# robotseu/ORB_Line_SLAM

Hardware: AMD Instinct MI355X
Metric: stereo frames/s extract+match (ORB+LBD), KITTI 1242x375 (higher is better)
Workload: dtype u8; 1 GPU; C3: 1242x375 stereo, 2000 ORB + 500 LBD per image, extract + stereo point/line match + f2f LBD match + SearchByBoW vs the previous frame (synthetic k=10 L=6 vocabulary, ComputeBoW included); parallelism=frame-sharded x1, distinct_pairs=512, order=shuffled, scene=default

## Files before the change

### orb_line_slam_amd/csrc/api.cpp

```cpp
#include "ctx.hpp"
#include "staging.hpp"
#include <map>
#include <mutex>

namespace olf {
static thread_local std::string g_err;
void set_error(const std::string& s) { g_err = s; }

int check_device(const olf_ctx* c, const char* who)
{
    int d = -1;
    if (hipGetDevice(&d) != hipSuccess || d != c->device) { set_error(std::string(who) + ": the context belongs to another device than the current one"); return OLF_ERR_INVALID; }
    return OLF_OK;
}

int scratch_get(olf_ctx* c, ScratchSlot slot, size_t bytes, void** out)
{
    if (c->scratch_bytes[slot] < bytes) {
        if (c->scratch[slot]) { OLF_HIP_CHECK(hipDeviceSynchronize()); (void)hipFree(c->scratch[slot]); c->scratch[slot] = nullptr; c->scratch_bytes[slot] = 0; }
        size_t want = std::max<size_t>(bytes * 3 / 2, 4096);
        OLF_HIP_CHECK(hipMalloc(&c->scratch[slot], want));
        c->scratch_bytes[slot] = want;
    }
    *out = c->scratch[slot];
// ... 171 lines not shown
    if (c->ev_join) (void)hipEventDestroy(c->ev_join);
    if (c->stream2) (void)hipStreamDestroy(c->stream2);
    if (c->stream) (void)hipStreamDestroy(c->stream);
    delete c;
}

int olf_ctx_create(const olf_params* p, int width, int height, int max_images, olf_ctx** out)
{
    if (!p || !out || width < 64 || height < 64 || max_images < 1) { set_error("olf_ctx_create: bad argument"); return OLF_ERR_INVALID; }
    *out = nullptr;
    if (p->abi_version != OLF_ABI_VERSION || p->struct_size != (uint32_t)sizeof(olf_params)) {
        set_error("olf_ctx_create: the parameter block was not initialised by this library's olf_default_params() (abi_version / struct_size differ: "
                  "caller built against another include/orbline_types.h)");
        return OLF_ERR_INVALID;
    }
    int ndev = 0;
    if (hipGetDeviceCount(&ndev) != hipSuccess || ndev < 1) {
        set_error("olf_ctx_create: no HIP device visible (this library has no CPU path)");
        return OLF_ERR_NODEVICE;
    }
    olf_ctx* c = new olf_ctx();
    c->params = *p; c->W = width; c->H = height; c->max_images = max_images;
    int rc = c->orb.build(p->orb, width, height);
    if (rc != OLF_OK) {
        set_error(rc == OLF_ERR_CAPACITY ? "olf_ctx_create: more than 32760 key points on one pyramid level (nfeatures too large for this scale factor / level count)"
                  : (width > kMaxOrbSide || height > kMaxOrbSide) ? "olf_ctx_create: image wider or higher than 4131 pixels (FAST candidates are packed with 12 bits per coordinate)"
                                         : "olf_ctx_create: image size / ORB parameters not supported (every pyramid level needs at least 62 x 62 pixels and a landscape cell grid)");
        delete c; return rc;
    }
    auto fail = [&](int code) { olf_ctx_destroy(c); return code; };
    if (hipGetDevice(&c->device) != hipSuccess) return fail(OLF_ERR_HIP);
    if (hipDeviceGetAttribute(&c->limits.nCU, hipDeviceAttributeMultiprocessorCount, c->device) != hipSuccess || c->limits.nCU <= 0) c->limits.nCU = 64;
    if (hipDeviceGetAttribute(&c->limits.maxLds, hipDeviceAttributeMaxSharedMemoryPerBlock, c->device) != hipSuccess) c->limits.maxLds = 64 * 1024;
    if (hipStreamCreateWithFlags(&c->stream, hipStreamNonBlocking) != hipSuccess) { set_error("hipStreamCreate failed"); return fail(OLF_ERR_HIP); }
    const OrbGeom& g = c->orb.geom;
    const size_t n = (size_t)max_images;
    OrbDeviceBufs& b = c->ob;
    const bool allocTrace = getenv("OLF_ALLOC_TRACE") != nullptr;
#define A(ptr, count) do { if ((rc = dev_alloc(c, &(ptr), (count))) != OLF_OK) return fail(rc); \
                           if (allocTrace) fprintf(stderr, "alloc %-18s %8.3f MB per image\n", #ptr, (double)(count) * sizeof(*(ptr)) / 1e6 / (double)n); } while (0)
    A(b.pyr, n * g.pyrBytes); A(b.blur, n * g.pyrBytes);
    A(b.cells, n * g.totalCells * g.cellCap); A(b.cellCount, n * g.totalCells);
    A(b.cand, n * g.candTotal); A(b.candNode, n * g.candTotal); A(b.candCount, n * g.nlevels);
    if (g.maxNodes > 2048) A(b.octSpill, n * g.nlevels * octree_lds_bytes(g.maxNodes));
    A(b.lvlKp, n * g.kpTotal); A(b.lvlCount, n * g.nlevels); A(b.lvlAngle, n * g.kpTotal);
    A(b.rx, c->orb.rx.size() + 1); A(b.ry, c->orb.ry.size() + 1); A(b.geom, 1); A(b.status, 256);
    A(c->d_sad, ((n + 1) / 2) * g.outCap); A(c->d_bestkey, ((n + 1) / 2) * g.outCap); A(c->d_rowperm, n * g.outCap);
    A(c->d_images, n * width * height);
#undef A
    if (hipMemcpy(b.rx, c->orb.rx.data(), c->orb.rx.size() * sizeof(ResizeCoef), hipMemcpyHostToDevice) != hipSuccess ||
        hipMemcpy(b.ry, c->orb.ry.data(), c->orb.ry.size() * sizeof(ResizeCoef), hipMemcpyHostToDevice) != hipSuccess ||
        hipMemcpy(b.geom, &g, sizeof(OrbGeom), hipMemcpyHostToDevice) != hipSuccess ||
        hipMemset(b.status, 0, 1024) != hipSuccess) {
        set_error("olf_ctx_create: table upload failed");
        return fail(OLF_ERR_HIP);
    }
    rc = c->line.build(p->line, width, height, max_images);
    if (rc != OLF_OK) { set_error("olf_ctx_create: LSD parameters not supported"); return fail(rc); }
    LineGeom& lg = c->line.geom;
    int prLeast = 0, prGreatest = 0;
    (void)hipDeviceGetStreamPriorityRange(&prLeast, &prGreatest);
    if (hipStreamCreateWithPriority(&c->stream2, hipStreamNonBlocking, prLeast) != hipSuccess ||
        hipEventCreateWithFlags(&c->ev_fork, hipEventDisableTiming) != hipSuccess || hipEventCreateWithFlags(&c->ev_front, hipEventDisableTiming) != hipSuccess || hipEventCreateWithFlags(&c->ev_sort, hipEventDisableTiming) != hipSuccess ||
        hipEventCreateWithFlags(&c->ev_lbd, hipEventDisableTiming) != hipSuccess ||
        hipEventCreateWithFlags(&c->ev_join, hipEventDisableTiming) != hipSuccess) { set_error("stream/event creation failed"); return fail(OLF_ERR_HIP); }
    LineDeviceBufs& l = c->lb;
#define A(ptr, count) do { if ((rc = dev_alloc(c, &(ptr), (count))) != OLF_OK) return fail(rc); \
                           if (allocTrace) fprintf(stderr, "alloc %-18s %8.3f MB per image\n", #ptr, (double)(count) * sizeof(*(ptr)) / 1e6 / (double)n); } while (0)
    const bool batchCtx = n > (size_t)kBatchCtxImages;
    const size_t keyWords = lg.wide ? 2 : 1;
    A(l.grad, n * lg.Ps); A(l.keysA, n * lg.Ps * keyWords); A(l.keysB, n * lg.Ps * keyWords);
    if (batchCtx && lg.Ps * 4 >= lg.pitchW * lg.H && lg.Ps * 4 >= lg.pitchS * lg.Hs) { l.lsdBlur = reinterpret_cast<uint8_t*>(l.keysA); l.scaled = reinterpret_cast<uint8_t*>(l.keysB); c->scaled_aliased = true; }
    else { A(l.lsdBlur, n * lg.pitchW * lg.H); A(l.scaled, n * lg.pitchS * lg.Hs); }
    A(l.topBuf, n * (size_t)lsd_seedsort_top_words()); A(l.keyCount, n * 32); A(l.maxN, n * 32); A(l.chunkCnt, n * ((lg.Ps + 4095) / 4096)); A(l.sortHist, n * (size_t)lsd_sort_max_chunks(lg.Ps) * 32); A(l.sortBase, n * 32);
    l.nChunks = lg.regionStride / 32;
    A(l.region, n * (size_t)lg.regionStride); l.ownerImages = (batchCtx || lg.wide) ? 0 : (int)std::min<size_t>(n, kMwMaxImages); A(l.owner, (size_t)l.ownerImages * lg.Ps); A(l.links, n * (size_t)l.nChunks);
    lg.logCap = lg.regionStride / 2;
    lg.spillBlocks = lg.regionStride / 2 >= lg.Ps ? 0 : (int)std::max<size_t>(4, n / 16);
    if (lg.spillBlocks) A(lg.spillArena, (size_t)lg.spillBlocks * 2 * lg.Ps);
    A(lg.spillCtl, 64); A(lg.spillOf, n);
    l.mgImages = (int)std::min<size_t>(n, kMgMaxImages); l.mgStride = lsd_grow_mg_stride(lg.maxRegions);
    A(l.mg, (size_t)l.mgImages * l.mgStride);
    A(l.rawLines, n * lg.maxDetect); A(l.rawCount, n); A(l.regCount, n); A(l.growFmt, n); A(l.lbdBlur, n * lg.pitchW * lg.H); A(l.dxdy, n * lg.pitchD * lg.H);
    A(l.rowSums, n * lg.outCap * 63 * 4); A(l.lbdStarts, n * lg.outCap * 64 * 2); A(l.rx, c->line.rx.size()); A(l.ry, c->line.ry.size()); A(l.geom, 1);
    A(c->d_ldist, ((n + 1) / 2) * lg.outCap * lg.outCap); A(c->d_lm21, ((n + 1) / 2) * lg.outCap);
    if (hipMalloc(&c->d_lprep, stereo_lines_prep_bytes((int)n, lg.outCap)) != hipSuccess) { set_error("hipMalloc failed"); return fail(OLF_ERR_HIP); }
    c->allocs.push_back(c->d_lprep);
    const bool slab = n <= 16;
    if (slab) {
        size_t off = 0;
        for (int k = 0; k < FB_FIELDS; ++k) { c->outslab_off[k] = off; off += (fb_bytes(c, k, n) + 255) & ~(size_t)255; }
        c->outslab_bytes = off;
        A(c->d_outslab, off);
        if (hipHostMalloc(reinterpret_cast<void**>(&c->h_outslab), off, hipHostMallocDefault) != hipSuccess) { set_error("hipHostMalloc failed"); return fail(OLF_ERR_HIP); }
    }
    for (int k = 0; k < FB_FIELDS; ++k) {
        uint8_t* q = nullptr;
        if (slab) q = c->d_outslab + c->outslab_off[k];
        else if ((rc = dev_alloc(c, &q, fb_bytes(c, k, n))) != OLF_OK) return fail(rc);
        fb_set_field(c->d_out, k, q);
        if (allocTrace) fprintf(stderr, "alloc %-18s %8.3f MB per image\n", kFrameFields[k].name, (double)fb_bytes(c, k, n) / 1e6 / (double)n);
    }
#undef A
    l.status = b.status;
    if (hipMemcpy(l.rx, c->line.rx.data(), c->line.rx.size() * sizeof(ResizeCoef), hipMemcpyHostToDevice) != hipSuccess ||
        hipMemcpy(l.ry, c->line.ry.data(), c->line.ry.size() * sizeof(ResizeCoef), hipMemcpyHostToDevice) != hipSuccess ||
        hipMemcpy(l.geom, &lg, sizeof(LineGeom), hipMemcpyHostToDevice) != hipSuccess) { set_error("line table upload failed"); return fail(OLF_ERR_HIP); }
    if ((rc = angle_tables_acquire(c->device, p->line.conv_libm_float, l, c->stream)) != OLF_OK) return fail(rc);
    c->has_tables = true;
    *out = c;
    return OLF_OK;
}

int olf_ctx_synchronize(olf_ctx* c)
{
    if (!c) return OLF_ERR_INVALID;
    OLF_HIP_CHECK(hipStreamSynchronize(c->stream));
    OLF_HIP_CHECK(hipStreamSynchronize(c->stream2));
    c->join_pending = false;
    return check_status(c);
}

int olf_ctx_set_input_event(olf_ctx* c, void* hip_event)
{
    if (!c) return OLF_ERR_INVALID;
    c->input_event = static_cast<hipEvent_t>(hip_event);
    return OLF_OK;
}

int olf_ctx_poll_status(olf_ctx* c)
{
    if (!c) return OLF_ERR_INVALID;
    return check_status(c);
}

int olf_profile_enable(olf_ctx* c, int on)
{
    if (!c) return OLF_ERR_INVALID;
    c->prof_on = on != 0;
    return OLF_OK;
}

static int prof_collect(olf_ctx* c)
{
    OLF_HIP_CHECK(hipDeviceSynchronize());
    for (auto& r : c->prof_recs) {
        float ms = 0;
        if (hipEventElapsedTime(&ms, r.a, r.b) == hipSuccess) { c->prof_ms[r.stage] += ms; c->prof_calls[r.stage] += 1; }
        c->prof_pool.push_back(r.a); c->prof_pool.push_back(r.b);
    }
    c->prof_recs.clear();
    return OLF_OK;
}

int olf_profile_reset(olf_ctx* c)
{
    if (!c) return OLF_ERR_INVALID;
    OLF_TRY(prof_collect(c));
    for (int i = 0; i < 16; ++i) { c->prof_ms[i] = 0; c->prof_calls[i] = 0; }
    return OLF_OK;
}

int olf_profile_stage_count(void) { return ST_COUNT; }
const char* olf_profile_stage_name(int i) { return (i >= 0 && i < ST_COUNT) ? kStageNames[i] : ""; }

int olf_profile_read(olf_ctx* c, double* total_ms, int32_t* calls)
{
// ... 323 lines not shown
```

### orb_line_slam_amd/csrc/lbd.hip

```cpp
#include "line_internal.hpp"
#include "device_math.hpp"

namespace olf {

#define OLF_TRY_RC(expr) do { int _rc = (expr); if (_rc != OLF_OK) return _rc; } while (0)

__constant__ int8_t c_bandPairs[64] = {
#include "lbd_band_pairs.inc"
};

constexpr int LS_LDS_KEYS = 4096;

template <typename P>
__device__ __forceinline__ void ls_bitonic_desc(P sk, int sortN, int tid)
{
    for (int k = 2; k <= sortN; k <<= 1)
        for (int j = k >> 1; j > 0; j >>= 1) {
            for (int i = tid; i < sortN; i += 256) {
                const int ixj = i ^ j;
                if (ixj > i) {
                    const unsigned long long a = sk[i], b = sk[ixj];
                    const bool desc = (i & k) == 0;
                    if (desc ? (a < b) : (a > b)) { sk[i] = b; sk[ixj] = a; }
                }
            }
            __syncthreads();
        }
}

__global__ __launch_bounds__(256) void k_line_select(const LineGeom* __restrict__ gp, const olf_keyline* __restrict__ rawLines,
                                                     const int* __restrict__ rawCount, olf_keyline* __restrict__ kls, int* __restrict__ counts,
                                                     unsigned long long* __restrict__ scratchAll, size_t scratchStride)
{
    extern __shared__ unsigned long long skeys[];
    const LineGeom& g = *gp;
    const int img = blockIdx.x, tid = threadIdx.x;
    const int R = min(rawCount[img], g.maxDetect);
    const olf_keyline* raw = rawLines + (size_t)img * g.maxDetect;
    olf_keyline* out = kls + (size_t)img * g.outCap;
    if (!(R > g.nFeatures && g.nFeatures != 0)) {
        const int n = min(R, g.outCap);
        for (int i = tid; i < n; i += 256) out[i] = raw[i];
        if (tid == 0) counts[img] = n;
        return;
    }
    int sortN = 64;
    while (sortN < R) sortN <<= 1;
    const bool inLds = sortN <= LS_LDS_KEYS;
    unsigned long long* gk = scratchAll + (size_t)img * scratchStride;
    for (int i = tid; i < sortN; i += 256) {
        unsigned long long k = 0;
        if (i < R) k = ((unsigned long long)__float_as_uint(raw[i].response) << 32) | (unsigned long long)(0xffffffffu - (unsigned)i);
        if (inLds) skeys[i] = k; else gk[i] = k;
    }
    __syncthreads();
    if (inLds) ls_bitonic_desc(skeys, sortN, tid); else ls_bitonic_desc(gk, sortN, tid);
    for (int i = tid; i < g.nFeatures; i += 256) {
        const unsigned idx = 0xffffffffu - (unsigned)((inLds ? skeys[i] : gk[i]) & 0xffffffffull);
        olf_keyline kl = raw[idx];
        kl.class_id = i;
        out[i] = kl;
    }
    if (tid == 0) counts[img] = g.nFeatures;
}

__global__ __launch_bounds__(256) void k_sobel3(const uint8_t* __restrict__ blur, uint32_t* __restrict__ dxdy, const LineGeom* __restrict__ gp)
{
    const LineGeom& g = *gp;
    const int img = blockIdx.y;
    const int wo = (g.W + 7) >> 3;
    const int t = blockIdx.x * 256 + threadIdx.x;
    if (t >= wo * g.H) return;
    const int y = t / wo, x0 = (t - y * wo) * 8;
    const uint8_t* b = blur + (size_t)img * g.pitchW * g.H;
    const int ym = y == 0 ? 1 : y - 1, yp = y == g.H - 1 ? g.H - 2 : y + 1;
    int v[3][10];
    const int rows[3] = {ym, y, yp};
#pragma unroll
    for (int r = 0; r < 3; ++r) {
        const uint8_t* row = b + (size_t)rows[r] * g.pitchW;
        const uint32_t w1 = *reinterpret_cast<const uint32_t*>(row + x0);
        const uint32_t w2 = x0 + 4 < g.pitchW ? *reinterpret_cast<const uint32_t*>(row + x0 + 4) : 0u;
        const uint32_t w0 = x0 > 0 ? *reinterpret_cast<const uint32_t*>(row + x0 - 4) : 0u;
        const uint32_t w3 = x0 + 8 < g.pitchW ? *reinterpret_cast<const uint32_t*>(row + x0 + 8) : 0u;
        v[r][0] = (int)(w0 >> 24);
#pragma unroll
        for (int k = 0; k < 4; ++k) { v[r][1 + k] = (int)((w1 >> (8 * k)) & 0xffu); v[r][5 + k] = (int)((w2 >> (8 * k)) & 0xffu); }
        v[r][9] = (int)(w3 & 0xffu);
        if (x0 == 0) v[r][0] = v[r][2];
#pragma unroll
        for (int k = 0; k < 8; ++k)
            if (x0 + k == g.W - 1) v[r][k + 2] = v[r][k];
    }
    uint32_t o[8];
#pragma unroll
    for (int k = 0; k < 8; ++k) {
        const int dx = (v[0][k + 2] - v[0][k]) + 2 * (v[1][k + 2] - v[1][k]) + (v[2][k + 2] - v[2][k]);
        const int dy = (v[2][k] + 2 * v[2][k + 1] + v[2][k + 2]) - (v[0][k] + 2 * v[0][k + 1] + v[0][k + 2]);
        o[k] = ((uint32_t)dx & 0xffffu) | ((uint32_t)dy << 16);
    }
    uint32_t* out = dxdy + (size_t)img * g.pitchD * g.H + (size_t)y * g.pitchD + x0;
    if (x0 < g.pitchD) *reinterpret_cast<uint4*>(out) = make_uint4(o[0], o[1], o[2], o[3]);
    if (x0 + 4 < g.pitchD) *reinterpret_cast<uint4*>(out + 4) = make_uint4(o[4], o[5], o[6], o[7]);
}

__global__ __launch_bounds__(64) void k_lbd_prep(const LineGeom* __restrict__ gp, const olf_keyline* __restrict__ kls, const int* __restrict__ counts,
                                                 float2* __restrict__ starts)
{
    const LineGeom& g = *gp;
    const int img = blockIdx.y, li = blockIdx.x * 64 + threadIdx.x;
    if (li >= counts[img]) return;
    const olf_keyline kl = kls[(size_t)img * g.outCap + li];
    const short heightOfLSP = 63;
    const short lengthOfLSP = (short)kl.numOfPixels;
    const short halfWidth = (short)((lengthOfLSP - 1) / 2);
    const short halfHeight = (short)((heightOfLSP - 1) / 2);
    const float midX = (float)(0.5 * (double)f_add(kl.sPointInOctaveX, kl.ePointInOctaveX));
    const float midY = (float)(0.5 * (double)f_add(kl.sPointInOctaveY, kl.ePointInOctaveY));
    const float dL0 = g.libmFloat ? glibc_cosf(kl.angle) : (float)cos((double)kl.angle);
    const float dL1 = g.libmFloat ? glibc_sinf(kl.angle) : (float)sin((double)kl.angle);
    float sCorX0 = f_add(f_add(f_mul(-dL0, (float)halfWidth), f_mul(dL1, (float)halfHeight)), midX);
    float sCorY0 = f_add(f_sub(f_mul(-dL1, (float)halfWidth), f_mul(dL0, (float)halfHeight)), midY);
    float2* o = starts + ((size_t)img * g.outCap + li) * 64;
    for (int h = 0; h < 63; ++h) {
        o[h] = make_float2(sCorX0, sCorY0);
        sCorX0 = f_sub(sCorX0, dL1); sCorY0 = f_add(sCorY0, dL0);
    }
    o[63] = make_float2(dL0, dL1);
}

constexpr int LR_U = 16, LR_P = LR_U + 1;
template <bool LEAN>
__global__ __launch_bounds__(256) void k_lbd_rows(const LineGeom* __restrict__ gp, const uint32_t* __restrict__ dxdyAll,
                                                  const olf_keyline* __restrict__ kls, const int* __restrict__ counts,
                                                  const float2* __restrict__ starts, float4* __restrict__ rowSums)
{
    __shared__ uint32_t s_t[4][64 * LR_P];
    const LineGeom& g = *gp;
    const int img = blockIdx.y, wv = threadIdx.x >> 6, lane = threadIdx.x & 63;
    const int li = blockIdx.x * 4 + wv;
    if (li >= counts[img]) return;
    const bool rowAct = lane < 63;
    const int hID = rowAct ? lane : 62;
    const uint32_t* dxdy = dxdyAll + (size_t)img * g.pitchD * g.H;
    const short lengthOfLSP = (short)kls[(size_t)img * g.outCap + li].numOfPixels;
    const int realWidth = g.pitchD;
    const short imageWidth = (short)(g.W - 1), imageHeight = (short)(g.H - 1);
    const float2* st = starts + ((size_t)img * g.outCap + li) * 64;
    const float2 dL = st[63], s0 = st[hID];
    const float dL0 = dL.x, dL1 = dL.y;
    const float dO0 = -dL1, dO1 = dL0;
    float sCorX = s0.x, sCorY = s0.y;
    float pgdL = 0, ngdL = 0, pgdO = 0, ngdO = 0;
    const bool flat = fabsf(dL0) >= fabsf(dL1);
    uint32_t* tb = s_t[wv];
    constexpr int U = LR_U;
    for (int w0 = 0; w0 < lengthOfLSP; w0 += U) {
        uint32_t p[U];
        int off[U];
#pragma unroll
        for (int u = 0; u < U; ++u) {
            int xCor, yCor;
            if (LEAN) {
                const float rx = __builtin_rintf(sCorX), ry = __builtin_rintf(sCorY);
                const float bx = f_sub(sCorX, rx) == 0.5f ? f_add(rx, 1.0f) : rx, by = f_sub(sCorY, ry) == 0.5f ? f_add(ry, 1.0f) : ry;
                xCor = min(max((int)bx, 0), (int)imageWidth); yCor = min(max((int)by, 0), (int)imageHeight);
            } else {
            int tc = (int)(short)roundf(sCorX);
            xCor = tc < 0 ? 0 : (tc > imageWidth ? imageWidth : tc);
            tc = (int)(short)roundf(sCorY);
            yCor = tc < 0 ? 0 : (tc > imageHeight ? imageHeight : tc);
            }
            off[u] = yCor * realWidth + xCor;
            sCorX = f_add(sCorX, dL0);
            sCorY = f_add(sCorY, dL1);
        }
        if (flat) {
#pragma unroll
            for (int u = 0; u < U; ++u) tb[lane * LR_P + u] = (uint32_t)off[u];
            __builtin_amdgcn_wave_barrier();
            const int a0 = (lane >> 4) * LR_P + (lane & 15);
            uint32_t v[16];
#pragma unroll
            for (int k = 0; k < 16; ++k) v[k] = dxdy[tb[a0 + 4 * k * LR_P]];
#pragma unroll
            for (int k = 0; k < 16; ++k) tb[a0 + 4 * k * LR_P] = v[k];
            __builtin_amdgcn_wave_barrier();
#pragma unroll
            for (int u = 0; u < U; ++u) p[u] = tb[lane * LR_P + u];
            __builtin_amdgcn_wave_barrier();
        } else {
#pragma unroll
            for (int u = 0; u < U; ++u) p[u] = dxdy[off[u]];
        }
#pragma unroll
        for (int u = 0; u < U; ++u) {
            if (w0 + u < lengthOfLSP) {
                const float dx = (float)(int)(int16_t)(p[u] & 0xffffu), dy = (float)(int)(int16_t)(p[u] >> 16);
                const float gDL = f_add(f_mul(dx, dL0), f_mul(dy, dL1));
                const float gDO = f_add(f_mul(dx, dO0), f_mul(dy, dO1));
                pgdL = f_add(pgdL, fmaxf(gDL, 0.f)); ngdL = f_sub(ngdL, fminf(gDL, 0.f));
                pgdO = f_add(pgdO, fmaxf(gDO, 0.f)); ngdO = f_sub(ngdO, fminf(gDO, 0.f));
            }
        }
    }
    if (rowAct) {
        const float cg = g.gaussCoefG[hID];
        rowSums[((size_t)img * g.outCap + li) * 63 + hID] = make_float4(f_mul(cg, pgdL), f_mul(cg, ngdL), f_mul(cg, pgdO), f_mul(cg, ngdO));
    }
}

__global__ __launch_bounds__(64) void k_lbd_desc(const LineGeom* __restrict__ gp, const float4* __restrict__ rowSums,
                                                 const int* __restrict__ counts, uint8_t* __restrict__ desc)
{
    const LineGeom& g = *gp;
    const int img = blockIdx.y;
    const int li = blockIdx.x * 64 + threadIdx.x;
    if (li >= counts[img]) return;
    const float4* rs = rowSums + ((size_t)img * g.outCap + li) * 63;
    float bs[9][8];
#pragma unroll
    for (int b = 0; b < 9; ++b)
#pragma unroll
        for (int k = 0; k < 8; ++k) bs[b][k] = 0.f;
// ... 22 lines not shown
                }
        }
    }
    float d[72];
    const float invN2 = (float)(1.0 / (7 * 2.0)), invN3 = (float)(1.0 / (7 * 3.0));
#pragma unroll
    for (int b = 0; b < 9; ++b) {
        const float invN = (b == 0 || b == 8) ? invN2 : invN3;
        float temp = f_mul(bs[b][0], invN);
        d[8 * b] = temp;
        d[8 * b + 4] = (float)sqrt((double)f_sub(f_mul(bs[b][2], invN), f_mul(temp, temp)));
        temp = f_mul(bs[b][1], invN);
        d[8 * b + 1] = temp;
        d[8 * b + 5] = (float)sqrt((double)f_sub(f_mul(bs[b][3], invN), f_mul(temp, temp)));
        temp = f_mul(bs[b][4], invN);
        d[8 * b + 2] = temp;
        d[8 * b + 6] = (float)sqrt((double)f_sub(f_mul(bs[b][6], invN), f_mul(temp, temp)));
        temp = f_mul(bs[b][5], invN);
        d[8 * b + 3] = temp;
        d[8 * b + 7] = (float)sqrt((double)f_sub(f_mul(bs[b][7], invN), f_mul(temp, temp)));
    }
    float tempM = 0, tempS = 0;
#pragma unroll
    for (int b = 0; b < 9; ++b) {
#pragma unroll
        for (int k = 0; k < 4; ++k) tempM = f_add(tempM, f_mul(d[8 * b + k], d[8 * b + k]));
#pragma unroll
        for (int k = 4; k < 8; ++k) tempS = f_add(tempS, f_mul(d[8 * b + k], d[8 * b + k]));
    }
    if (g.libmFloat) { tempM = f_div(1.0f, sqrtf(tempM)); tempS = f_div(1.0f, sqrtf(tempS)); }
    else { tempM = (float)(1 / sqrt((double)tempM)); tempS = (float)(1 / sqrt((double)tempS)); }
#pragma unroll
    for (int b = 0; b < 9; ++b) {
#pragma unroll
        for (int k = 0; k < 4; ++k) d[8 * b + k] = f_mul(d[8 * b + k], tempM);
#pragma unroll
        for (int k = 4; k < 8; ++k) d[8 * b + k] = f_mul(d[8 * b + k], tempS);
    }
#pragma unroll
    for (int i = 0; i < 72; ++i)
        if ((double)d[i] > 0.4) d[i] = (float)0.4;
    float temp = 0;
#pragma unroll
    for (int i = 0; i < 72; ++i) temp = f_add(temp, f_mul(d[i], d[i]));
    temp = g.libmFloat ? f_div(1.0f, sqrtf(temp)) : (float)(1 / sqrt((double)temp));
#pragma unroll
    for (int i = 0; i < 72; ++i) d[i] = f_mul(d[i], temp);
    uint8_t* o = desc + ((size_t)img * g.outCap + li) * OLF_DESC_BYTES;
#pragma unroll
    for (int c = 0; c < 32; ++c) {
        const int p = c_bandPairs[2 * c], q = c_bandPairs[2 * c + 1];
        unsigned r = 0;
#pragma unroll
        for (int i = 0; i < 8; ++i) {
            float f1 = 0, f2 = 0;
#pragma unroll
            for (int bb = 0; bb < 9; ++bb) { if (bb == p) f1 = d[8 * bb + i]; if (bb == q) f2 = d[8 * bb + i]; }
            if (f1 > f2) r += 1u << i;
        }
        o[c] = (uint8_t)r;
    }
}

int launch_lbd_dense(const LineGeom& g, const LineDeviceBufs& b, const uint8_t* d_in, int in_pitch, int n_images, hipStream_t s)
{
    OLF_TRY_RC(launch_gauss7_img(d_in, in_pitch, (size_t)in_pitch * g.H, b.lbdBlur, g.pitchW, (size_t)g.pitchW * g.H, g.W, g.H, g, 1, n_images, s));
    hipLaunchKernelGGL(k_sobel3, dim3((((g.W + 7) >> 3) * g.H + 255) / 256, n_images), dim3(256), 0, s, b.lbdBlur, b.dxdy, b.geom);
    OLF_HIP_CHECK(hipGetLastError());
    return OLF_OK;
}

int launch_line_select(const LineGeom& g, const LineDeviceBufs& b, int n_images, olf_keyline* d_kls, int* d_counts, hipStream_t s)
{
    int sortN = 64;
    while (sortN < g.maxDetect) sortN <<= 1;
    hipLaunchKernelGGL(k_line_select, dim3(n_images), dim3(256), std::min(sortN, LS_LDS_KEYS) * sizeof(unsigned long long), s, b.geom, b.rawLines, b.rawCount, d_kls,
                       d_counts, reinterpret_cast<unsigned long long*>(b.keysA), (size_t)g.Ps / 2);
    OLF_HIP_CHECK(hipGetLastError());
    return OLF_OK;
}

int launch_lbd_desc(const LineGeom& g, const LineDeviceBufs& b, int n_images, const olf_keyline* d_kls, uint8_t* d_desc, const int* d_counts, hipStream_t s)
{
    hipLaunchKernelGGL(k_lbd_prep, dim3((g.outCap + 63) / 64, n_images), dim3(64), 0, s, b.geom, d_kls, d_counts, reinterpret_cast<float2*>(b.lbdStarts));
    if (g.W + 256 < 32768 && g.H + 256 < 32768)
        hipLaunchKernelGGL(k_lbd_rows<true>, dim3((g.outCap + 3) / 4, n_images), dim3(256), 0, s, b.geom, b.dxdy, d_kls, d_counts,
                           reinterpret_cast<const float2*>(b.lbdStarts), reinterpret_cast<float4*>(b.rowSums));
    else
        hipLaunchKernelGGL(k_lbd_rows<false>, dim3((g.outCap + 3) / 4, n_images), dim3(256), 0, s, b.geom, b.dxdy, d_kls, d_counts,
                           reinterpret_cast<const float2*>(b.lbdStarts), reinterpret_cast<float4*>(b.rowSums));
    hipLaunchKernelGGL(k_lbd_desc, dim3((g.outCap + 63) / 64, n_images), dim3(64), 0, s, b.geom, reinterpret_cast<const float4*>(b.rowSums),
                       d_counts, d_desc);
    OLF_HIP_CHECK(hipGetLastError());
    return OLF_OK;
}

}
```

### orb_line_slam_amd/csrc/line_internal.hpp

```cpp
#pragma once
#include "olf_internal.hpp"

namespace olf {

struct LineGeom {
    int W, H, pitchW;
    int Ws, Hs, pitchS, Ps;
    int nThr;
    int nBins;
    int wide;
    int minRegSize;
    double prec;
    double precWrap;
    double scale;
    double minLength;
    int maxDetect;
    int rectGrid;
    int maxRegions;
    int nFeatures;
    int outCap;
    int pitchD;
    int lsdTaps[7];
    int lsdWideR;
    int lsdWide[15];
    int lbdTaps[7];
    float gaussCoefL[21];
    float gaussCoefG[63];
    int resizeTabX, resizeTabY;
    int resizeTiled;
    int seedOrder;
    int refine;
    double densityTh;
    double logNT, logEps, pProb;
    int libmFloat;
    uint32_t divWsM; int divWsS;
    float alignTanLo, alignTanHi;
    float alignDeg;
    int regionStride;
    int resizeExact;
    int logCap;
    int spillBlocks;
    uint32_t* spillArena;
    int* spillCtl;
    int* spillOf;
};

struct LineDeviceBufs {
    uint8_t* lsdBlur = nullptr;
    uint8_t* scaled = nullptr;
    uint32_t* grad = nullptr;
    uint32_t* keysA = nullptr;
    uint32_t* keysB = nullptr;
    int* keyCount = nullptr;
    int* maxN = nullptr;
    int* chunkCnt = nullptr;
    uint32_t* region = nullptr;
    olf_keyline* rawLines = nullptr;
    int* rawCount = nullptr;
    int* regCount = nullptr;
    uint8_t* lbdBlur = nullptr;
    uint32_t* dxdy = nullptr;
    float* rowSums = nullptr;
    float* lbdStarts = nullptr;
    ResizeCoef* rx = nullptr;
    ResizeCoef* ry = nullptr;
    LineGeom* geom = nullptr;
    uint32_t* sortHist = nullptr;
    uint32_t* sortBase = nullptr;
    int* status = nullptr;
    float* angDeg = nullptr;
    void* angEnt = nullptr;
    int ownerImages = 0;
    uint32_t* owner = nullptr;
    int* links = nullptr;
    int nChunks = 0;
    int* growFmt = nullptr;
    int* topBuf = nullptr;
    unsigned char* mg = nullptr;
    size_t mgStride = 0;
    int mgImages = 0;
};

struct LsdOverrides {
    int sortMode = -1;
    int waves = -1, robEntries = 0;
    int groups = -1;
    int poolChunks = 0;
    int scatter = 0;
};

struct DeviceLimits { int nCU = 64, maxLds = 64 * 1024; };

struct LsdPlan {
    enum Resize { Upgrad, Tiled, Upsample } resize;
    enum Sort { Radix, Seed, Wide } sort;
    bool keysOwner, keysAll;
    int sortWaves;
    bool sortTop; int sortGroups;
    int growWaves;
    int robEntries, growGroups, poolChunks, scatter;
    int agentRefine, agentPF, agentLaunches;
    enum Rect { Emit, Mixed, Plain } rect;
};
LsdPlan lsd_plan(const LineGeom& g, const LineDeviceBufs& b, const LsdOverrides& o, const DeviceLimits& d, int n_images);

constexpr int kBatchCtxImages = 2048;

struct LineHostTables {
    LineGeom geom;
    std::vector<ResizeCoef> rx, ry;
    int build(const olf_line_params& p, int W, int H, int max_images = 2);
};

int launch_lsd_dense(const LineGeom& g, const LineDeviceBufs& b, const LsdPlan& p, const uint8_t* d_in, int in_pitch, int n_images, hipStream_t s, bool writeScaled);
int launch_lsd_seed_order(const LineGeom& g, const LineDeviceBufs& b, const LsdPlan& p, int n_images, hipStream_t s);
int launch_lsd_grow(const LineGeom& g, const LineDeviceBufs& b, const LsdPlan& p, int n_images, hipStream_t s);
int launch_lsd_rect(const LineGeom& g, const LineDeviceBufs& b, const LsdPlan& p, int n_images, hipStream_t s);
int launch_line_select(const LineGeom& g, const LineDeviceBufs& b, int n_images, olf_keyline* d_kls, int* d_counts, hipStream_t s);
int launch_lbd_dense(const LineGeom& g, const LineDeviceBufs& b, const uint8_t* d_in, int in_pitch, int n_images, hipStream_t s);
int launch_lbd_desc(const LineGeom& g, const LineDeviceBufs& b, int n_images, const olf_keyline* d_kls, uint8_t* d_desc, const int* d_counts, hipStream_t s);
int launch_gauss7_img(const uint8_t* src, int srcPitch, size_t srcStride, uint8_t* dst, int dstPitch, size_t dstStride, int W, int H,
                      const LineGeom& g, int which, int n_images, hipStream_t s);
int launch_lsd_angle_table(LineDeviceBufs& b, int libmFloat, hipStream_t s);
int launch_fdiv_sweep(unsigned long long seed, int blocks, int per_thread, unsigned long long* d_mismatches, hipStream_t s);
int launch_sqrtq_sweep(int count, unsigned long long* d_mismatches, hipStream_t s);
int launch_align_sweep(const LineDeviceBufs& b, unsigned long long seed, int blocks, int per_thread, unsigned long long* d_out, hipStream_t s);
int lsd_sort_max_chunks(int Ps);
size_t lsd_grow_mg_stride(int maxRegions);
constexpr int kMwMaxImages = 3072;
constexpr int kMgMaxImages = 64;
int launch_lsd_grow_mw(const LineGeom& g, const LineDeviceBufs& b, const LsdPlan& p, int n_images, hipStream_t s);
int lsd_seedsort_top_words();
int launch_lsd_sort(const LineGeom& g, const LineDeviceBufs& b, int n_images, hipStream_t s);
int launch_lsd_seedsort(const LineGeom& g, const LineDeviceBufs& b, const LsdPlan& p, int n_images, hipStream_t s, int nOverride, int kthrOverride, int depthOverride);
int launch_lsd_sort_wide(const LineGeom& g, const LineDeviceBufs& b, int n_images, hipStream_t s, int nOverride, long long kthrOverride, int depthOverride, int fullOverride);

size_t stereo_lines_prep_bytes(int n_images, int cap);
int launch_stereo_lines(int W, int H, const olf_stereo_params& P, int n_pairs, const olf_keyline* d_kls, const uint8_t* d_desc,
                        const int* d_counts, int cap, void* d_prep, uint16_t* d_dist , int* d_m21, int* d_m12,
                        float* d_disp, double* d_le, hipStream_t s);

}
```

### orb_line_slam_amd/csrc/lsd.hip

```cpp
#include "lsd_device.hpp"

namespace olf {


__device__ __forceinline__ int refl101(int p, int n)
{
    if (p < 0) p = -p;
    if (p >= n) p = 2 * (n - 1) - p;
    return p;
}

int launch_gauss7_img(const uint8_t* src, int srcPitch, size_t srcStride, uint8_t* dst, int dstPitch, size_t dstStride, int W, int H,
                      const LineGeom& g, int which, int n_images, hipStream_t s)
{
    if (!which && g.lsdWideR > 3) return launch_sep_wide(src, srcStride, srcPitch, dst, dstStride, dstPitch, W, H, g.lsdWide, g.lsdWideR, n_images, s);
    return launch_sep7(src, srcStride, srcPitch, dst, dstStride, dstPitch, W, H, which ? g.lbdTaps : g.lsdTaps, n_images, s);
}

__global__ __launch_bounds__(256) void k_lsd_upsample(const uint8_t* __restrict__ src, uint8_t* __restrict__ dst,
                                                      const LineGeom* __restrict__ gp, const ResizeCoef* __restrict__ rx,
                                                      const ResizeCoef* __restrict__ ry)
{
    const LineGeom& g = *gp;
    const int img = blockIdx.y;
    const int quads = (g.Ws + 3) >> 2;
    const int idx = blockIdx.x * 256 + threadIdx.x;
    if (idx >= quads * g.Hs) return;
    const int dy = idx / quads, dx0 = (idx - dy * quads) * 4;
    const uint8_t* s = src + (size_t)img * g.pitchW * g.H;
    const ResizeCoef cy = ry[dy];
    const int y0 = min(max((int)cy.ofs, 0), g.H - 1), y1 = min(max((int)cy.ofs + 1, 0), g.H - 1);
    const uint8_t* S0 = s + (size_t)y0 * g.pitchW;
    const uint8_t* S1 = s + (size_t)y1 * g.pitchW;
    const int b0 = cy.a0, b1 = cy.a1;
    uint32_t out = 0;
#pragma unroll
    for (int k = 0; k < 4; ++k) {
        const int dx = dx0 + k;
        if (dx < g.Ws) {
            const ResizeCoef cx = rx[dx];
            const int sx = cx.ofs, sx1 = min(sx + 1, g.W - 1);
            const int h0 = S0[sx] * cx.a0 + S0[sx1] * cx.a1;
            const int h1 = S1[sx] * cx.a0 + S1[sx1] * cx.a1;
            const int v = g.resizeExact ? (h0 * b0 + h1 * b1 + 32768) >> 16 : (((b0 * (h0 >> 4)) >> 16) + ((b1 * (h1 >> 4)) >> 16) + 2) >> 2;
            out |= (uint32_t)(v & 0xff) << (8 * k);
        }
    }
    *reinterpret_cast<uint32_t*>(dst + (size_t)img * g.pitchS * g.Hs + (size_t)dy * g.pitchS + dx0) = out;
}

constexpr int LG_CHUNK = 4096;
__global__ __launch_bounds__(256) void k_lsd_grad(const uint8_t* __restrict__ scaled, uint32_t* __restrict__ grad,
                                                  const LineGeom* __restrict__ gp, int* __restrict__ maxN, int* __restrict__ chunkCnt)
{
    __shared__ int s_max[4], s_def[4];
    const LineGeom& g = *gp;
    const int img = blockIdx.y;
    int n = 0, ndef = 0;
    const uint8_t* sc = scaled + (size_t)img * g.pitchS * g.Hs;
    uint32_t* gout = grad + (size_t)img * g.Ps;
#pragma unroll 2
    for (int k = 0; k < LG_CHUNK / 1024; ++k) {
        const int idx0 = blockIdx.x * LG_CHUNK + (k * 256 + threadIdx.x) * 4;
        if (idx0 >= g.Ps) break;
        const int y = idx0 / g.Ws, x = idx0 - y * g.Ws;
        uint32_t packed[4] = {kNotDef, kNotDef, kNotDef, kNotDef};
        if (idx0 + 3 < g.Ps && x + 8 <= g.Ws && y < g.Hs - 1) {
            const uint8_t* r0 = sc + (size_t)y * g.pitchS + x;
            unsigned long long w0, w1;
            __builtin_memcpy(&w0, r0, 8);
            __builtin_memcpy(&w1, r0 + g.pitchS, 8);
#pragma unroll
            for (int p = 0; p < 4; ++p) {
                const int A = (int)((w0 >> (8 * p)) & 0xff), B = (int)((w0 >> (8 * p + 8)) & 0xff);
                const int C = (int)((w1 >> (8 * p)) & 0xff), D = (int)((w1 >> (8 * p + 8)) & 0xff);
                const int DA = D - A, BC = B - C;
                const int gx = DA + BC, gy = DA - BC;
                const int nn = gx * gx + gy * gy;
                if (nn >= g.nThr) { packed[p] = pack_g(gx, gy); n = max(n, nn); ++ndef; }
                else packed[p] = pack_g(gx, gy) | kNotDef;
            }
        } else {
            int yy = y, xx = x;
// ... 78 lines not shown
            const int dy = dy0 + rr;
            if (dy > dh || (rr > 0 && dy - 1 >= dh)) break;
            int n0, n1;
            uint32_t c0, c1;
            rows_of(dy + 1, n0, n1, c0, c1);
            Raw q0 = p0, q1 = p1;
            if (rr < UG_ROWS) {
                if (n0 != r0 && n0 != r1) q0 = load_row(n0);
                if (n1 != n0 && n1 != r1) q1 = load_row(n1);
                __builtin_amdgcn_sched_barrier(0);
            }
            uint32_t h0[5], h1[5];
            if (r0 == ra) { for (int k = 0; k < 5; ++k) h0[k] = hA[k]; }
            else if (r0 == rb) { for (int k = 0; k < 5; ++k) h0[k] = hB[k]; }
            else hrow(p0, h0);
            if (r1 == r0) { for (int k = 0; k < 5; ++k) h1[k] = h0[k]; }
            else if (r1 == rb) { for (int k = 0; k < 5; ++k) h1[k] = hB[k]; }
            else hrow(p1, h1);
            int cur[5];
#pragma unroll
            for (int k = 0; k < 5; ++k) cur[k] = (int)(((((b0 * h0[k]) >> 16) + ((b1 * h1[k]) >> 16) + 2u) >> 2) & 0xffu);
            if (writeScaled && rr < UG_ROWS && dy < dh) {
                const uint32_t out = (uint32_t)cur[0] | ((uint32_t)cur[1] << 8) | ((uint32_t)cur[2] << 16) | ((uint32_t)cur[3] << 24);
                __builtin_memcpy(d + (size_t)dy * g.pitchS, &out, 4);
            }
            if (rr > 0) {
                const int y = dy - 1;
                uint32_t packed[4];
#pragma unroll
                for (int k = 0; k < 4; ++k) {
                    const int A = prev[k], B = prev[k + 1], Cc = cur[k], D = cur[k + 1];
                    const int DA = D - A, BC = B - Cc;
                    const int gx = DA + BC, gy = DA - BC;
                    const int nn = gx * gx + gy * gy;
                    const bool inside = dx0 + k < dw - 1 && y < dh - 1;
                    packed[k] = inside ? (pack_g(gx, gy) | (nn >= g.nThr ? 0u : kNotDef)) : kNotDef;
                    if (inside && nn >= g.nThr) nmax = max(nmax, nn);
                }
                uint32_t* o = gout + (size_t)y * dw + dx0;
                const uintptr_t oa = reinterpret_cast<uintptr_t>(o);
                if (dx0 + 3 < dw && (oa & 15) == 0) *reinterpret_cast<uint4*>(o) = make_uint4(packed[0], packed[1], packed[2], packed[3]);
                else if (dx0 + 3 < dw && (oa & 7) == 0) {
                    reinterpret_cast<uint2*>(o)[0] = make_uint2(packed[0], packed[1]); reinterpret_cast<uint2*>(o)[1] = make_uint2(packed[2], packed[3]);
                } else {
#pragma unroll
                    for (int k = 0; k < 4; ++k) if (dx0 + k < dw) o[k] = packed[k];
                }
            }
#pragma unroll
            for (int k = 0; k < 5; ++k) prev[k] = cur[k];
            ra = r0; rb = r1;
#pragma unroll
            for (int k = 0; k < 5; ++k) { hA[k] = h0[k]; hB[k] = h1[k]; }
            r0 = n0; r1 = n1; b0 = c0; b1 = c1; p0 = q0; p1 = q1;
        }
    }
#pragma unroll
    for (int o = 32; o > 0; o >>= 1) nmax = max(nmax, __shfl_xor(nmax, o));
    if (threadIdx.x == 0 && nmax > 0) atomicMax(&maxN[img * 32], nmax);
}

constexpr int KEYS_THREADS = 512;
__device__ __forceinline__ int lsd_bin(int n, double bin_coef, float bin_coef_half_f)
{
    const float tf = __builtin_amdgcn_sqrtf((float)n) * bin_coef_half_f;
    const int b = (int)tf;
    const float fr = tf - (float)b;
    if (n != 0 && (fr < 1e-3f || fr > 0.999f)) return (int)(sqrt_quarter(n) * bin_coef);
    return b;
}

template <bool OWNER, bool ALLKEYS, int CH, bool WIDE = false>
__global__ __launch_bounds__(KEYS_THREADS) void k_lsd_keys(uint32_t* __restrict__ gradAll, const LineGeom* __restrict__ gp,
                                                  const int* __restrict__ maxN, const int* __restrict__ chunkCnt, uint32_t* __restrict__ keys,
                                                  int* __restrict__ keyCount, uint32_t* __restrict__ owner, const float* __restrict__ angDeg,
                                                  int nChunks, int total)
{
    constexpr int NWV = KEYS_THREADS / 64, SPAN = CH / NWV;
    extern __shared__ float s_deg[];
    __shared__ uint16_t s_list[CH];
    __shared__ int s_wcnt[NWV], s_base;
    const LineGeom& g = *gp;
    const int lane = threadIdx.x & 63, wv = threadIdx.x >> 6;
    const int L = blockIdx.x, per = total >> 3;
    const int V = L < per * 8 ? (L & 7) * per + (L >> 3) : L;
    const int img = V / nChunks, chunk = V - img * nChunks;
    const int Ws = g.Ws, Hs = g.Hs, Ps = g.Ps, nBins1 = g.nBins - 1;
    const uint32_t divM = g.divWsM, divS = g.divWsS;
    const float alignDeg = g.alignDeg;
    const double precG = g.prec;
    uint32_t* grad = gradAll + (size_t)img * Ps;
    const int c0 = chunk * CH;
    const int lo = c0 - Ws - 1, hi = c0 + CH + Ws + 1;
    const float kNaN = __builtin_nanf("");
    if (threadIdx.x == 0) s_base = 0;
    const double max_grad = sqrt((double)maxN[img * 32] / 4.0);
    const double bin_coef = (max_grad > 0) ? (double)nBins1 / max_grad : 0;
    const float bin_coef_half_f = 0.5f * (float)bin_coef;
    constexpr int NB = 8;
    constexpr bool SPLIT = ALLKEYS && !WIDE && CH == NB * KEYS_THREADS;
    if (SPLIT) {
        uint32_t* kall = keys + (size_t)img * Ps;
        const int keyEnd = min(Ps, (Hs - 1) * Ws);
        {
            uint32_t p[NB];
            float d[NB];
#pragma unroll
            for (int u = 0; u < NB; ++u) { const int idx = c0 + (int)threadIdx.x + u * KEYS_THREADS; p[u] = idx < Ps ? grad[idx] : kNotDef; }
#pragma unroll
            for (int u = 0; u < NB; ++u) d[u] = (p[u] & kNotDef) ? kNaN : angDeg[p[u] & 0x3fffffu];
#pragma unroll
            for (int u = 0; u < NB; ++u) s_deg[Ws + 1 + (int)threadIdx.x + u * KEYS_THREADS] = d[u];
#pragma unroll
            for (int u = 0; u < NB; ++u) {
                const int idx = c0 + (int)threadIdx.x + u * KEYS_THREADS;
                const int y = (int)(__umulhi((uint32_t)idx, divM) >> divS), x = idx - y * Ws;
                const int gx = unpack_gx(p[u]), gy = unpack_gy(p[u]);
                const int n = gx * gx + gy * gy;
                const float tf = __builtin_amdgcn_sqrtf((float)n) * bin_coef_half_f;
                int bin = (int)tf;
                const float fr = tf - (float)bin;
                const bool valid = (idx < keyEnd) & (x < Ws - 1);
                if (valid & (n != 0) & ((fr < 1e-3f) | (fr > 0.999f))) bin = (int)(sqrt_quarter(n) * bin_coef);
                if (valid) kall[(uint32_t)(idx - y)] = ((uint32_t)(nBins1 - bin) << 22) | (uint32_t)idx;
            }
        }
#pragma unroll
        for (int side = 0; side < 2; ++side) {
            const int first = side ? c0 + CH : lo, qBase = side ? CH + Ws + 1 : 0;
            constexpr int NH = 4;
            for (int h0 = (int)threadIdx.x; h0 < Ws + 1; h0 += NH * KEYS_THREADS) {
                uint32_t p[NH];
                float d[NH];
#pragma unroll
                for (int u = 0; u < NH; ++u) { const int h = h0 + u * KEYS_THREADS, idx = first + h; p[u] = (h < Ws + 1) & ((unsigned)idx < (unsigned)Ps) ? grad[idx] : kNotDef; }
#pragma unroll
                for (int u = 0; u < NH; ++u) d[u] = (p[u] & kNotDef) ? kNaN : angDeg[p[u] & 0x3fffffu];
#pragma unroll
                for (int u = 0; u < NH; ++u) if (h0 + u * KEYS_THREADS < Ws + 1) s_deg[qBase + h0 + u * KEYS_THREADS] = d[u];
            }
        }
    } else
    for (int i0 = lo + (int)threadIdx.x; i0 < hi; i0 += NB * KEYS_THREADS) {
        uint32_t p[NB];
        float d[NB];
#pragma unroll
        for (int u = 0; u < NB; ++u) { const int idx = i0 + u * KEYS_THREADS; p[u] = (unsigned)idx < (unsigned)Ps && idx < hi ? grad[idx] : kNotDef; }
#pragma unroll
        for (int u = 0; u < NB; ++u) d[u] = (p[u] & kNotDef) ? kNaN : angDeg[p[u] & 0x3fffffu];
#pragma unroll
        for (int u = 0; u < NB; ++u) if (i0 + u * KEYS_THREADS < hi) s_deg[i0 + u * KEYS_THREADS - lo] = d[u];
        if (ALLKEYS) {
            uint32_t* kall = keys + (size_t)img * Ps;
            unsigned long long* kallW = reinterpret_cast<unsigned long long*>(keys) + (size_t)img * Ps;
#pragma unroll
            for (int u = 0; u < NB; ++u) {
                const int idx = i0 + u * KEYS_THREADS;
                if (idx >= c0 && idx < min(Ps, c0 + CH)) {
                    const int y = WIDE ? idx / Ws : (int)(__umulhi((uint32_t)idx, divM) >> divS), x = idx - y * Ws;
                    if (x < Ws - 1 && y < Hs - 1) {
                        const int gx = unpack_gx(p[u]), gy = unpack_gy(p[u]);
                        if (WIDE) {
                            const int bin = (int)(sqrt_quarter(gx * gx + gy * gy) * bin_coef);
                            kallW[(size_t)y * (Ws - 1) + x] = ((unsigned long long)(uint32_t)(nBins1 - bin) << 32) | (unsigned long long)(uint32_t)idx;
                        } else {
                        const int bin = lsd_bin(gx * gx + gy * gy, bin_coef, bin_coef_half_f);
                        kall[y * (Ws - 1) + x] = ((uint32_t)(nBins1 - bin) << 22) | (uint32_t)idx;
                        }
// ... 1341 lines not shown
```

### orb_line_slam_amd/csrc/orb_describe.hip

```cpp
#include "olf_internal.hpp"
#include "device_math.hpp"

namespace olf {

__constant__ __attribute__((aligned(16))) int8_t c_pattern[1024] = {
#include "orb_pattern_31.inc"
};

constexpr int DESC_KPW = 1;

__global__ __launch_bounds__(256) void k_describe(const OrbGeom* __restrict__ gp, const uint8_t* __restrict__ pyr,
                                                  const uint8_t* __restrict__ blur, const uint32_t* __restrict__ lvlKp,
                                                  const int* __restrict__ lvlCount, olf_keypoint* __restrict__ kps,
                                                  uint8_t* __restrict__ desc, int* __restrict__ counts, int out_cap,
                                                  int* __restrict__ status)
{
    constexpr int PR = 18, PW = 2 * PR + 1, PDW = 10;
    __shared__ float4 s_patf[256];
    __shared__ uint32_t s_w0[256], s_w1[256];
    __shared__ uint32_t s_patch[4][PW * PDW];
    const OrbGeom& g = *gp;
    const int img = blockIdx.y, lane = threadIdx.x & 63, wv = threadIdx.x >> 6;
    {
        const uint32_t pw = reinterpret_cast<const uint32_t*>(c_pattern)[threadIdx.x];
        s_patf[threadIdx.x] = make_float4((float)(int8_t)(pw & 0xff), (float)(int8_t)((pw >> 8) & 0xff), (float)(int8_t)((pw >> 16) & 0xff), (float)(int8_t)(pw >> 24));
    }
    {
        const int r = threadIdx.x >> 3, j = threadIdx.x & 7, v = r - kHalfPatch;
        uint32_t w0 = 0, w1 = 0;
        if (r <= 2 * kHalfPatch) {
            const int d = g.umax[v < 0 ? -v : v];
#pragma unroll
            for (int b = 0; b < 4; ++b) {
                const int u = 4 * j + b - 16;
                if (u >= -d && u <= d) { w0 |= 1u << (8 * b); w1 |= (uint32_t)(u + 16) << (8 * b); }
            }
        }
        s_w0[threadIdx.x] = w0; s_w1[threadIdx.x] = w1;
    }
    __syncthreads();
    const int nlevels = g.nlevels, kpTotal = g.kpTotal;
    const int* lc = lvlCount + img * nlevels;
    if (blockIdx.x == 0 && threadIdx.x == 0) {
        int tot = 0;
        for (int l = 0; l < nlevels; ++l) tot += lc[l];
        if (tot > out_cap) { atomicOr(status, 4); tot = out_cap; }
        counts[img] = tot;
    }
    const int nbx = (int)gridDim.x, per = nbx >> 3;
    const int vblock = ((int)blockIdx.x < per * 8) ? ((int)blockIdx.x & 7) * per + ((int)blockIdx.x >> 3) : (int)blockIdx.x;
    const int r6 = lane / PDW, c10 = lane - r6 * PDW;
    uint32_t* patch = s_patch[wv];
#pragma unroll 1
    for (int q = 0; q < DESC_KPW; ++q) {
        const int slot = (vblock * 4 + wv) * DESC_KPW + q;
        if (slot >= kpTotal) break;
        const uint32_t p = lvlKp[(size_t)img * kpTotal + slot];
        const bool lv_lane = lane < nlevels;
        const int base_l = lv_lane ? g.lv[lane].kpBase : 0x7fffffff, cnt_l = lv_lane ? lc[lane] : 0;
        const int level = (int)__popcll(wave_vote(lv_lane && lane > 0 && slot >= base_l));
        const int i = slot - __builtin_amdgcn_readlane(base_l, level);
        if (i >= __builtin_amdgcn_readlane(cnt_l, level)) continue;
        const int outIdx = i + wave_sum_i32(lane < level ? cnt_l : 0);
        if (outIdx >= out_cap) continue;
        const LevelGeom& L = g.lv[level];
        const int cx = (int)(p >> 20) + kMinBorder, cy = (int)((p >> 8) & 0xfff) + kMinBorder, score = (int)(p & 0xff);
        const int pitch = L.pitch;

        const uint8_t* bl = blur + (size_t)img * g.pyrBytes + L.offset;
        const int x0 = (cx - PR) & ~3, xs = cx - x0;
        uint32_t stg[(PW + 5) / 6];
        {
            const int xo = min(x0 + 4 * c10, pitch - 4);
            const uint32_t stBase = (uint32_t)((cy - PR + r6) * pitch + xo);
#pragma unroll
            for (int k = 0; k < (PW + 5) / 6; ++k) {
                stg[k] = 0u;
                if (lane < 60 && 6 * k + r6 < PW) stg[k] = *reinterpret_cast<const uint32_t*>(bl + (stBase + (uint32_t)(6 * k * pitch)));
            }
        }

        const uint8_t* im = pyr + (size_t)img * g.pyrBytes + L.offset;
        int m10 = 0, m01 = 0, sI = 0;
        const uint32_t icBase = (uint32_t)((cy - kHalfPatch + (lane >> 3)) * pitch + cx - 16 + 4 * (lane & 7));
#pragma unroll
        for (int pass = 0; pass < 4; ++pass) {
            if (pass * 64 + lane < (2 * kHalfPatch + 1) * 8) {
                uint32_t I;
                __builtin_memcpy(&I, im + (icBase + (uint32_t)(pass * 8 * pitch)), 4);
                const int rs = (int)__builtin_amdgcn_udot4(I, s_w0[pass * 64 + lane], 0u, false);
                m10 = (int)__builtin_amdgcn_udot4(I, s_w1[pass * 64 + lane], (uint32_t)m10, false);
                sI += rs;
                m01 += (pass * 8 + (lane >> 3) - kHalfPatch) * rs;
            }
        }
        m10 -= 16 * sI;
        m10 = wave_sum_i32(m10);
        m01 = wave_sum_i32(m01);
        const float angle = dev_fastAtan2((float)m01, (float)m10);

        const float factorPI = (float)(3.1415926535897932384626433832795 / 180.f);
        const float rad = __fmul_rn(angle, factorPI);
        const float a = glibc_cosf(rad), b = glibc_sinf(rad);
        __builtin_amdgcn_wave_barrier();
#pragma unroll
        for (int k = 0; k < (PW + 5) / 6; ++k)
            if (lane < 60 && 6 * k + r6 < PW) patch[60 * k + lane] = stg[k];
        __builtin_amdgcn_wave_barrier();
        const uint8_t* pb = reinterpret_cast<const uint8_t*>(patch) + PR * (PDW * 4) + xs;
        unsigned long long bits[4];
#pragma unroll
        for (int j = 0; j < 4; ++j) {
            const float4 pt = s_patf[j * 64 + lane];
            const int r0 = __float2int_rn(__fadd_rn(__fmul_rn(pt.x, b), __fmul_rn(pt.y, a)));
            const int c0 = __float2int_rn(__fsub_rn(__fmul_rn(pt.x, a), __fmul_rn(pt.y, b)));
            const int r1 = __float2int_rn(__fadd_rn(__fmul_rn(pt.z, b), __fmul_rn(pt.w, a)));
            const int c1 = __float2int_rn(__fsub_rn(__fmul_rn(pt.z, a), __fmul_rn(pt.w, b)));
            const int t0 = pb[r0 * (PDW * 4) + c0], t1 = pb[r1 * (PDW * 4) + c1];
            bits[j] = wave_vote(t0 < t1);
        }
        if (lane == 0) {
            unsigned long long* d = reinterpret_cast<unsigned long long*>(desc + ((size_t)img * out_cap + outIdx) * OLF_DESC_BYTES);
            d[0] = bits[0]; d[1] = bits[1]; d[2] = bits[2]; d[3] = bits[3];
            olf_keypoint k;
            k.x = (float)cx; k.y = (float)cy;
            if (level != 0) { k.x = __fmul_rn(k.x, L.scale); k.y = __fmul_rn(k.y, L.scale); }
            k.size = (float)L.patch_size; k.angle = angle; k.response = (float)score; k.octave = level; k.class_id = -1;
            kps[(size_t)img * out_cap + outIdx] = k;
        }
    }
}

int launch_orb_describe(const OrbGeom& g, const OrbDeviceBufs& b, int n_images, olf_keypoint* d_kps, uint8_t* d_desc,
// ... 10 lines not shown
```

Before: 14920 stereo frames/s.

## Sort LBD lines by row and remap row-sum blocks across XCDs for locality

k_lbd_prep now ranks each image's keylines by their midpoint y coordinate with an O(n^2) rank pass in LDS and writes a permutation. k_lbd_rows processes lines in that order over a flattened 1D grid, with blocks remapped so that contiguous line ranges land on the same XCD. The goal is to improve L2 reuse of the dxdy gradient rows, since neighbouring lines touch overlapping image rows. The existing XCD remap helper is also factored into a shared header. The costs are the quadratic ranking in the prep kernel and one extra indirection per line.

```diff
diff --git a/orb_line_slam_amd/csrc/api.cpp b/orb_line_slam_amd/csrc/api.cpp
--- a/orb_line_slam_amd/csrc/api.cpp
+++ b/orb_line_slam_amd/csrc/api.cpp
@@ -277,7 +277,7 @@
     l.mgImages = (int)std::min<size_t>(n, kMgMaxImages); l.mgStride = lsd_grow_mg_stride(lg.maxRegions);
     A(l.mg, (size_t)l.mgImages * l.mgStride);
     A(l.rawLines, n * lg.maxDetect); A(l.rawCount, n); A(l.regCount, n); A(l.growFmt, n); A(l.lbdBlur, n * lg.pitchW * lg.H); A(l.dxdy, n * lg.pitchD * lg.H);
-    A(l.rowSums, n * lg.outCap * 63 * 4); A(l.lbdStarts, n * lg.outCap * 64 * 2); A(l.rx, c->line.rx.size()); A(l.ry, c->line.ry.size()); A(l.geom, 1);
+    A(l.rowSums, n * lg.outCap * 63 * 4); A(l.lbdStarts, n * lg.outCap * 64 * 2); A(l.lbdOrder, n * lg.outCap); A(l.rx, c->line.rx.size()); A(l.ry, c->line.ry.size()); A(l.geom, 1);
     A(c->d_ldist, ((n + 1) / 2) * lg.outCap * lg.outCap); A(c->d_lm21, ((n + 1) / 2) * lg.outCap);
     if (hipMalloc(&c->d_lprep, stereo_lines_prep_bytes((int)n, lg.outCap)) != hipSuccess) { set_error("hipMalloc failed"); return fail(OLF_ERR_HIP); }
     c->allocs.push_back(c->d_lprep);
diff --git a/orb_line_slam_amd/csrc/lbd.hip b/orb_line_slam_amd/csrc/lbd.hip
--- a/orb_line_slam_amd/csrc/lbd.hip
+++ b/orb_line_slam_amd/csrc/lbd.hip
@@ -1,5 +1,6 @@
 #include "line_internal.hpp"
 #include "device_math.hpp"
+#include "xcd_order.hpp"
 
 namespace olf {
 
@@ -104,12 +105,33 @@
     if (x0 + 4 < g.pitchD) *reinterpret_cast<uint4*>(out + 4) = make_uint4(o[4], o[5], o[6], o[7]);
 }
 
+constexpr int LP_MAX_KEYS = 8192;
 __global__ __launch_bounds__(64) void k_lbd_prep(const LineGeom* __restrict__ gp, const olf_keyline* __restrict__ kls, const int* __restrict__ counts,
-                                                 float2* __restrict__ starts)
-{
+                                                 float2* __restrict__ starts, int* __restrict__ order)
+{
+    extern __shared__ int s_key[];
     const LineGeom& g = *gp;
     const int img = blockIdx.y, li = blockIdx.x * 64 + threadIdx.x;
-    if (li >= counts[img]) return;
+    const int count = min(counts[img], g.outCap);
+    if (blockIdx.x * 64 >= count) return;
+    const bool ranked = count <= LP_MAX_KEYS;
+    if (ranked) {
+        for (int j = threadIdx.x; j < count; j += 64) {
+            const olf_keyline& kj = kls[(size_t)img * g.outCap + j];
+            s_key[j] = min(max((int)(0.5f * (kj.sPointInOctaveY + kj.ePointInOctaveY)), 0), g.H - 1);
+        }
+        __syncthreads();
+    }
+    if (li >= count) return;
+    {
+        int rank = li;
+        if (ranked) {
+            const int key = s_key[li];
+            rank = 0;
+            for (int j = 0; j < count; ++j) { const int kj = s_key[j]; rank += (kj < key || (kj == key && j < li)) ? 1 : 0; }
+        }
+        order[(size_t)img * g.outCap + rank] = li;
+    }
     const olf_keyline kl = kls[(size_t)img * g.outCap + li];
     const short heightOfLSP = 63;
     const short lengthOfLSP = (short)kl.numOfPixels;
@@ -133,13 +155,16 @@
 template <bool LEAN>
 __global__ __launch_bounds__(256) void k_lbd_rows(const LineGeom* __restrict__ gp, const uint32_t* __restrict__ dxdyAll,
                                                   const olf_keyline* __restrict__ kls, const int* __restrict__ counts,
-                                                  const float2* __restrict__ starts, float4* __restrict__ rowSums)
+                                                  const float2* __restrict__ starts, const int* __restrict__ order, float4* __restrict__ rowSums,
+                                                  int blocksPerImage, int total)
 {
     __shared__ uint32_t s_t[4][64 * LR_P];
     const LineGeom& g = *gp;
-    const int img = blockIdx.y, wv = threadIdx.x >> 6, lane = threadIdx.x & 63;
-    const int li = blockIdx.x * 4 + wv;
-    if (li >= counts[img]) return;
+    const int wv = threadIdx.x >> 6, lane = threadIdx.x & 63;
+    const int V = xcd_virtual_block((int)blockIdx.x, total);
+    const int img = V / blocksPerImage, slot = (V - img * blocksPerImage) * 4 + wv;
+    if (slot >= min(counts[img], g.outCap)) return;
+    const int li = order[(size_t)img * g.outCap + slot];
     const bool rowAct = lane < 63;
     const int hID = rowAct ? lane : 62;
     const uint32_t* dxdy = dxdyAll + (size_t)img * g.pitchD * g.H;
@@ -328,13 +353,18 @@
 
 int launch_lbd_desc(const LineGeom& g, const LineDeviceBufs& b, int n_images, const olf_keyline* d_kls, uint8_t* d_desc, const int* d_counts, hipStream_t s)
 {
-    hipLaunchKernelGGL(k_lbd_prep, dim3((g.outCap + 63) / 64, n_images), dim3(64), 0, s, b.geom, d_kls, d_counts, reinterpret_cast<float2*>(b.lbdStarts));
+    if (n_images <= 0) return OLF_OK;
+    const int blocksPerImage = (g.outCap + 3) / 4;
+    const long long total = (long long)blocksPerImage * n_images;
+    if (total > 0x7fffffffLL) { set_error("launch_lbd_desc: outCap / 4 x images exceeds the grid limit"); return OLF_ERR_CAPACITY; }
+    hipLaunchKernelGGL(k_lbd_prep, dim3((g.outCap + 63) / 64, n_images), dim3(64), (size_t)std::min(g.outCap, LP_MAX_KEYS) * sizeof(int), s, b.geom, d_kls, d_counts,
+                       reinterpret_cast<float2*>(b.lbdStarts), b.lbdOrder);
     if (g.W + 256 < 32768 && g.H + 256 < 32768)
-        hipLaunchKernelGGL(k_lbd_rows<true>, dim3((g.outCap + 3) / 4, n_images), dim3(256), 0, s, b.geom, b.dxdy, d_kls, d_counts,
-                           reinterpret_cast<const float2*>(b.lbdStarts), reinterpret_cast<float4*>(b.rowSums));
+        hipLaunchKernelGGL(k_lbd_rows<true>, dim3((unsigned)total), dim3(256), 0, s, b.geom, b.dxdy, d_kls, d_counts,
+                           reinterpret_cast<const float2*>(b.lbdStarts), b.lbdOrder, reinterpret_cast<float4*>(b.rowSums), blocksPerImage, (int)total);
     else
-        hipLaunchKernelGGL(k_lbd_rows<false>, dim3((g.outCap + 3) / 4, n_images), dim3(256), 0, s, b.geom, b.dxdy, d_kls, d_counts,
-                           reinterpret_cast<const float2*>(b.lbdStarts), reinterpret_cast<float4*>(b.rowSums));
+        hipLaunchKernelGGL(k_lbd_rows<false>, dim3((unsigned)total), dim3(256), 0, s, b.geom, b.dxdy, d_kls, d_counts,
+                           reinterpret_cast<const float2*>(b.lbdStarts), b.lbdOrder, reinterpret_cast<float4*>(b.rowSums), blocksPerImage, (int)total);
     hipLaunchKernelGGL(k_lbd_desc, dim3((g.outCap + 63) / 64, n_images), dim3(64), 0, s, b.geom, reinterpret_cast<const float4*>(b.rowSums),
                        d_counts, d_desc);
     OLF_HIP_CHECK(hipGetLastError());
diff --git a/orb_line_slam_amd/csrc/line_internal.hpp b/orb_line_slam_amd/csrc/line_internal.hpp
--- a/orb_line_slam_amd/csrc/line_internal.hpp
+++ b/orb_line_slam_amd/csrc/line_internal.hpp
@@ -62,6 +62,7 @@
     uint32_t* dxdy = nullptr;
     float* rowSums = nullptr;
     float* lbdStarts = nullptr;
+    int* lbdOrder = nullptr;
     ResizeCoef* rx = nullptr;
     ResizeCoef* ry = nullptr;
     LineGeom* geom = nullptr;
diff --git a/orb_line_slam_amd/csrc/lsd.hip b/orb_line_slam_amd/csrc/lsd.hip
--- a/orb_line_slam_amd/csrc/lsd.hip
+++ b/orb_line_slam_amd/csrc/lsd.hip
@@ -1,4 +1,5 @@
 #include "lsd_device.hpp"
+#include "xcd_order.hpp"
 
 namespace olf {
 
@@ -243,8 +244,7 @@
     __shared__ int s_wcnt[NWV], s_base;
     const LineGeom& g = *gp;
     const int lane = threadIdx.x & 63, wv = threadIdx.x >> 6;
-    const int L = blockIdx.x, per = total >> 3;
-    const int V = L < per * 8 ? (L & 7) * per + (L >> 3) : L;
+    const int V = xcd_virtual_block((int)blockIdx.x, total);
     const int img = V / nChunks, chunk = V - img * nChunks;
     const int Ws = g.Ws, Hs = g.Hs, Ps = g.Ps, nBins1 = g.nBins - 1;
     const uint32_t divM = g.divWsM, divS = g.divWsS;
diff --git a/orb_line_slam_amd/csrc/orb_describe.hip b/orb_line_slam_amd/csrc/orb_describe.hip
--- a/orb_line_slam_amd/csrc/orb_describe.hip
+++ b/orb_line_slam_amd/csrc/orb_describe.hip
@@ -1,5 +1,6 @@
 #include "olf_internal.hpp"
 #include "device_math.hpp"
+#include "xcd_order.hpp"
 
 namespace olf {
 
@@ -47,8 +48,7 @@
         if (tot > out_cap) { atomicOr(status, 4); tot = out_cap; }
         counts[img] = tot;
     }
-    const int nbx = (int)gridDim.x, per = nbx >> 3;
-    const int vblock = ((int)blockIdx.x < per * 8) ? ((int)blockIdx.x & 7) * per + ((int)blockIdx.x >> 3) : (int)blockIdx.x;
+    const int vblock = xcd_virtual_block((int)blockIdx.x, (int)gridDim.x);
     const int r6 = lane / PDW, c10 = lane - r6 * PDW;
     uint32_t* patch = s_patch[wv];
 #pragma unroll 1
diff --git a/orb_line_slam_amd/csrc/xcd_order.hpp b/orb_line_slam_amd/csrc/xcd_order.hpp
--- /dev/null
+++ b/orb_line_slam_amd/csrc/xcd_order.hpp
@@ -0,0 +1,11 @@
+#pragma once
+
+namespace olf {
+
+__device__ __forceinline__ int xcd_virtual_block(int L, int total)
+{
+    const int per = total >> 3;
+    return L < per * 8 ? (L & 7) * per + (L >> 3) : L;
+}
+
+}
```

Measured after the change: 15010 stereo frames/s (median of 3 runs). Within noise of the previous version (+0.6%).
